# superyuri/FinRL

Hardware: AMD Instinct MI355X
Metric: env-steps/sec at N parallel envs (DOW30, 8 indicators) (higher is better)
Workload: dtype f64

## Files before the change

### finrl_amd/csrc/finenv_stock.hip

```cpp

#include "finenv_stock_common.h"

namespace {

constexpr int kAssetBatch = 16;
template <typename P>
__device__ __forceinline__ double end_total_asset(const P &p, const double *close, int E, int N, int e)
{
    const double *prow = close + (size_t)SI(FINENV_SI_PRICE_DAY) * N;
    double s = 0.0;
    for (int i0 = 0; i0 < N; i0 += kAssetBatch) {
        double pr[kAssetBatch];
        int hd[kAssetBatch];
#pragma unroll
        for (int j = 0; j < kAssetBatch; ++j) {
            const int i = min(i0 + j, N - 1);
            pr[j] = prow[i];
            hd[j] = HOLD(i);
        }
#pragma unroll
        for (int j = 0; j < kAssetBatch; ++j) {
            pin(pr[j]);
            pin(hd[j]);
        }
// ... 93 lines not shown
                    const int el = (N == 1) ? f : (int)__umulhi((unsigned)f, p.magicN);
                    const int kk = ks[el];
                    if (kk >= 1) p.h.actions[((size_t)(kk - 1) * E + e0) * N + f] = v[j];
                }
            }
        }
    }
    if (k >= 1) {
        p.h.asset[(size_t)k * E + e] = end_total_asset(p, p.close, E, N, e);
        p.h.row[(size_t)k * E + e] = SI(FINENV_SI_DAY);
        p.h.len[e] = k + 1;
    }
}

__global__ void stock_history_arm_kernel(const HistoryArgs p)
{
    const int E = p.E, N = p.N;
    const int e = blockIdx.x * blockDim.x + threadIdx.x;
    if (e >= E || (p.mask != nullptr && p.mask[e] == 0)) return;
    p.h.asset[e] = SI(FINENV_SI_DAY) == SI(FINENV_SI_START_DAY) ? SF(FINENV_SF_ASSET0)
                                                                : end_total_asset(p, p.close, E, N, e);
    p.h.row[e] = SI(FINENV_SI_DAY);
    p.h.len[e] = 1;
    p.h.flags[e] = 0;
}

}

struct finenv_stock : finenv_host::Handle {
    finenv_stock_config cfg;
    finenv_stock_panel panel;
    finenv_stock_state st;
    int obs_pitch;
    int desync_hint;
    uint32_t magicN;
    double *last;
    int32_t *win;
    int has_hist;
    finenv_stock_history hist;
    finenv_stock_impl::StepPlan plan;
};

namespace {

Params make_params(const finenv_stock *h)
{
    Params p;
    memset(&p, 0, sizeof(p));
    p.cfg = h->cfg;
    p.panel = h->panel;
    p.st = h->st;
    p.D = h->D;
    p.obs_pitch = h->obs_pitch;
    p.desync_hint = h->desync_hint;
    p.magicN = h->magicN;
    p.last = h->last;
    p.win = h->win;
    return p;
}

int launch_aux(finenv_stock *h, const Params &p, int mode, hipStream_t stream)
{
    if (h->cfg.n_tickers <= 32) finenv_stock_impl::launch_aux_np32(p, mode, stream);
    else if (h->cfg.n_tickers <= 64) finenv_stock_impl::launch_aux_np64(p, mode, stream);
    else finenv_stock_impl::launch_aux_np128(p, mode, stream);
    return 0;
}

void plan_step(finenv_stock *h)
{
    const bool win = h->win != nullptr, desync = h->desync_hint != 0;
    const int N = h->cfg.n_tickers;
    finenv_stock_impl::StepPlan &pl = h->plan;
    pl = N <= 32   ? finenv_stock_impl::choose_step_np32(h->cfg, win, desync)
         : N <= 64 ? finenv_stock_impl::choose_step_np64(h->cfg, win, desync)
                   : finenv_stock_impl::choose_step_np128(h->cfg, win, desync);
    const void *fn = reinterpret_cast<const void *>(pl.kernel);
    const finenv_host::DeviceGuard guard(h->device);
    int dev = h->device, cus = 0, per_cu = 0;
    if (dev < 0) (void)hipGetDevice(&dev);
    pl.lds_refused = pl.lds_bytes > 64 * 1024 &&
                     hipFuncSetAttribute(fn, hipFuncAttributeMaxDynamicSharedMemorySize, (int)pl.lds_bytes) != hipSuccess;
    if (hipDeviceGetAttribute(&cus, hipDeviceAttributeMultiprocessorCount, dev) != hipSuccess || cus < 1) cus = 256;
    if (hipOccupancyMaxActiveBlocksPerMultiprocessor(&per_cu, fn, kStepThreads, pl.lds_bytes) != hipSuccess || per_cu < 1)
        per_cu = 1;
    (void)hipGetLastError();
    pl.round = per_cu * cus;
}

void launch_step_rounds(const finenv_stock_impl::StepPlan &pl, const Params &p, hipStream_t stream)
{
    const int blocks = (p.cfg.n_envs + kWave - 1) / kWave;
    const int k = (blocks + pl.round - 1) / pl.round;
    const int chunk = k > 1 ? (blocks + k - 1) / k : blocks;
    Params q = p;
    int b = 0;
    do {
        q.block_base = b;
        const int nb = blocks - b < chunk ? blocks - b : chunk;
        hipLaunchKernelGGL(pl.kernel, dim3((unsigned)nb), dim3(kStepThreads), pl.lds_bytes, stream, q);
        b += chunk;
    } while (b < blocks);
}

HistoryArgs make_history_args(const finenv_stock *h)
{
    HistoryArgs a;
    memset(&a, 0, sizeof(a));
    a.h = h->hist;
    a.st = h->st;
    a.close = h->panel.close;
    a.E = h->cfg.n_envs;
    a.N = h->cfg.n_tickers;
    a.magicN = h->magicN;
    return a;
}

void launch_history_arm(const finenv_stock *h, const uint8_t *mask, hipStream_t stream)
{
    HistoryArgs a = make_history_args(h);
    a.mask = mask;
    hipLaunchKernelGGL(stock_history_arm_kernel, dim3((a.E + 255) / 256), dim3(256), 0, stream, a);
}

finenv_host::HistorySeries history_series(const finenv_stock *h)
{
    return {h->hist.asset, nullptr, nullptr, h->hist.len, h->hist.flags, 0, h->hist.capacity, h->cfg.n_envs};
}

}

#ifdef FINENV_DIAG
unsigned long long *g_finenv_dbg = nullptr;
#define g_dbg g_finenv_dbg
extern "C" void finenv_diag_set_stamp_buffer(void *ptr) { g_finenv_dbg = (unsigned long long *)ptr; }
#endif

extern "C" {

int finenv_abi_version(void) { return FINENV_ABI_VERSION; }

int finenv_struct_size(int which)
{
    switch (which) {
    case 0: return (int)sizeof(finenv_stock_config);
    case 1: return (int)sizeof(finenv_stock_panel);
    case 2: return (int)sizeof(finenv_stock_state);
    case 3: return (int)sizeof(finenv_portfolio_config);
    case 4: return (int)sizeof(finenv_portfolio_panel);
    case 5: return (int)sizeof(finenv_portfolio_state);
    case 6: return (int)sizeof(finenv_crypto_config);
    case 7: return (int)sizeof(finenv_crypto_panel);
    case 8: return (int)sizeof(finenv_crypto_state);
    case 9: return (int)sizeof(finenv_stocknp_config);
    case 10: return (int)sizeof(finenv_stocknp_panel);
    case 11: return (int)sizeof(finenv_stocknp_state);
    case 12: return (int)sizeof(finenv_cashpenalty_config);
    case 13: return (int)sizeof(finenv_cashpenalty_panel);
    case 14: return (int)sizeof(finenv_cashpenalty_state);
    case 15: return (int)sizeof(finenv_stoploss_config);
    case 16: return (int)sizeof(finenv_stoploss_panel);
    case 17: return (int)sizeof(finenv_stoploss_state);
    case 19: return (int)sizeof(finenv_btc_config);
    case 20: return (int)sizeof(finenv_btc_panel);
    case 21: return (int)sizeof(finenv_btc_state);
    case 23: return (int)sizeof(finenv_replay_view);
    case 24: return (int)sizeof(finenv_replay_batch);
    case 26: return (int)sizeof(finenv_replay_nstep);
    case 28: return (int)sizeof(finenv_replay_per);
    case 30: return (int)sizeof(finenv_rollout_view);
    case 31: return (int)sizeof(finenv_rollout_batch);
    case 33: return (int)sizeof(finenv_vecnorm);
    default: return FINENV_ERR_INVALID;
    }
}

const char *finenv_strerror(int code)
{
    switch (code) {
    case FINENV_OK: return "ok";
    case FINENV_ERR_INVALID: return "invalid argument";
    case FINENV_ERR_UNBOUND: return "panel/state not bound";
    case FINENV_ERR_HIP: return "HIP runtime error";
// ... 229 lines not shown
```

### finrl_amd/csrc/finenv_stock_common.h

```cpp
#pragma once
#include <hip/hip_runtime.h>
#include <stdint.h>
#include <stdio.h>
#include <stdlib.h>
#include <string.h>

#include <cstddef>
#include <new>
#include <type_traits>

#include "finenv.h"
#include "finenv_dev.h"
#include "finenv_host.h"

namespace finenv_stock_impl {
struct Params {
    finenv_stock_config cfg;
    finenv_stock_panel panel;
    finenv_stock_state st;
    const float *actions;
    float *obs;
    float *reward;
    uint8_t *done;
    float *term_obs;
    int32_t *realised;
    const uint8_t *mask;
    double *stats_out;
    int32_t auto_reset;
    int32_t D;
    int32_t obs_pitch;
    int32_t desync_hint;
    int32_t day0;
    uint32_t magicN;
    int32_t block_base;
    int32_t diag;
    unsigned long long *dbg;
    double *last;
    const int32_t *win;
};
}

namespace {

constexpr int kWave = 64;
constexpr int kStepThreads = 2 * kWave;

using finenv_stock_impl::Params;

#ifdef FINENV_DIAG
#define DIAG(bit) (p.diag & (bit))
#define STAMP(k)                                                                          \
    do {                                                                                  \
        if (p.dbg != nullptr && lane == 0) {                                              \
            __builtin_amdgcn_sched_barrier(0);                                            \
            p.dbg[((size_t)(blockIdx.x + p.block_base) * 2 + role) * 16 + (k)] = __builtin_amdgcn_s_memrealtime(); \
            __builtin_amdgcn_sched_barrier(0);                                            \
        }                                                                                 \
    } while (0)
#else
#define DIAG(bit) 0
#define STAMP(k) do { } while (0)
#endif

#define SF(fld) (*at(p.st.f64, (unsigned)(fld) * (unsigned)E + (unsigned)e))
#define SI(fld) (*at(p.st.i32, (unsigned)(fld) * (unsigned)E + (unsigned)e))
#define HOLD(i) SI(FINENV_STOCK_I32_FIELDS + (i))
#define SH0(i) SI(FINENV_STOCK_I32_FIELDS + N + (i))
#define SL(fld) (*at(p.last, (unsigned)(fld) * (unsigned)E + (unsigned)e))

__device__ __forceinline__ void latch_last_episode(const Params &p, double *last, int E, int e,
                                                   double end_asset)
{
#define LB(fld) (*at(last, (unsigned)(fld) * (unsigned)E + (unsigned)e))
    LB(FINENV_SL_COUNT) = LB(FINENV_SL_COUNT) + 1.0;
    LB(FINENV_SL_EPISODE) = (double)SI(FINENV_SI_EPISODE);
    LB(FINENV_SL_BEGIN_ASSET) = SF(FINENV_SF_ASSET0);
    LB(FINENV_SL_END_ASSET) = end_asset;
    LB(FINENV_SL_COST) = SF(FINENV_SF_COST);
    LB(FINENV_SL_TRADES) = (double)SI(FINENV_SI_TRADES);
    LB(FINENV_SL_RET_N) = (double)(SI(FINENV_SI_DAY) - SI(FINENV_SI_START_DAY));
    LB(FINENV_SL_RET_SUM) = SF(FINENV_SF_RET_SUM);
    LB(FINENV_SL_RET_SUMSQ) = SF(FINENV_SF_RET_SUMSQ);
#undef LB
}

__device__ __forceinline__ double *last_block()
{
    const char *ka = (const char *)__builtin_amdgcn_kernarg_segment_ptr();
    asm volatile("" : "+s"(ka));
    return *reinterpret_cast<double *const *>(ka + offsetof(Params, last));
}


__device__ __forceinline__ void ce(int &a, int &b)
{
    const int lo = min(a, b);
    const int hi = max(a, b);
    a = lo;
    b = hi;
}

}

namespace finenv_stock_impl {
struct StepPlan {
    void (*kernel)(Params);
    size_t lds_bytes;
    int round;
    int lds_refused;
};
StepPlan choose_step_np32(const finenv_stock_config &cfg, bool win, bool desync);
StepPlan choose_step_np64(const finenv_stock_config &cfg, bool win, bool desync);
StepPlan choose_step_np128(const finenv_stock_config &cfg, bool win, bool desync);
void launch_aux_np32(const Params &p, int mode, hipStream_t stream);
void launch_aux_np64(const Params &p, int mode, hipStream_t stream);
void launch_aux_np128(const Params &p, int mode, hipStream_t stream);
}
```

### finrl_amd/csrc/finenv_stock_kernels.inc

```

constexpr int kNPad = FINENV_NP;
constexpr int kLog2NPad = FINENV_LOG2NP;
constexpr bool kWide = kNPad > 32;
constexpr int kRow = kNPad + 1;
constexpr int kAuxWaves = kWide ? 1 : 4;
constexpr int kLdsPerWave = kWave * kRow;
constexpr int kAMax = kWide ? 1 << 23 : 1 << 25;
static_assert((long long)kAMax * kNPad + kNPad <= (1ll << 31), "keys must fit int32");
static_assert((1 << kLog2NPad) == kNPad, "NP must be a power of two");

__device__ __forceinline__ void sort_keys(int (&k)[kNPad])
{
#define CE(i, j) ce(k[i], k[j]);
#include FINENV_SORTNET
#undef CE
}


__device__ __forceinline__ double floordiv_exact(double a, double d)
{
    double x = __builtin_amdgcn_rcp(d);
    x = fma(fma(-d, x, 1.0), x, x);
    double q = floor(a * x);
    const double r = fma(-q, d, a);
// ... 148 lines not shown
        }
        for (int k = k_lo; k < nchunk; ++k) {
            const int col = k * kWave + lane;
            const int hidx = col - 1 - N;
            const bool in = col < D;
            const bool patch = in && (col == 0 || (hidx >= 0 && hidx < N));
            const int sel = (col == 0) ? 0 : (patch ? 1 + hidx : 0);
            const bool any_patch = __any(patch);
            for (int g = 0; g < nenv_w; g += kRows) {
                if (((lane_mask >> g) & 0xFFFFFFFFull) == 0ull) continue;
                float t[kRows];
#pragma unroll
                for (int j = 0; j < kRows; ++j) {
                    const int rd = __builtin_amdgcn_readlane(row_day, min(g + j, nenv_w - 1));
                    t[j] = *at(tmpl, (unsigned)(rd * D + (in ? col : 0)));
                }
#pragma unroll
                for (int j = 0; j < kRows; ++j) pin(t[j]);
#pragma unroll
                for (int j = 0; j < kRows; ++j) {
                    const int el = g + j;
                    if (el >= nenv_w || !((lane_mask >> el) & 1ull)) continue;
                    float v = t[j];
                    if (any_patch) {
                        const float pv = pfn(el, sel);
                        v = patch ? pv : v;
                    }
                    if (in) *at(base, (unsigned)(el * P + col)) = v;
                }
            }
        }
        return;
    }
    for (int k = k_lo; k < nchunk; ++k) {
        const int col = k * kWave + lane;
        const bool in = col < D;
        const int hidx = col - 1 - N;
        const bool patch = in && (col == 0 || (hidx >= 0 && hidx < N));
        const int sel = (col == 0) ? 0 : (patch ? 1 + hidx : 0);
        const bool any_patch = __any(patch);
        {
            const float t = in ? *at(tmpl, (unsigned)(rd0 * D + col)) : 0.0f;
            if (all_rows && !any_patch) {
#pragma unroll 8
                for (int el = 0; el < nenv_w; ++el)
                    if (in) *at(base, (unsigned)(el * P + col)) = t;
            } else if (all_rows) {
#pragma unroll 8
                for (int el = 0; el < nenv_w; ++el) {
                    const float pv = pfn(el, sel);
                    if (in) *at(base, (unsigned)(el * P + col)) = patch ? pv : t;
                }
            } else {
                for (int el = 0; el < nenv_w; ++el) {
                    if (!((lane_mask >> el) & 1ull)) continue;
                    const float pv = pfn(el, sel);
                    if (in) *at(base, (unsigned)(el * P + col)) = patch ? pv : t;
                }
            }
        }
    }
}

template <int kDesyncCh = 1>
__device__ __forceinline__ void write_obs_rows(float *__restrict__ dst,
                                               const float *__restrict__ tmpl, int D, int P, int N,
                                               int e0, int nenv_w, int row_day,
                                               unsigned long long lane_mask,
                                               const float *rows, int lane, int k_lo = 0,
                                               int k_hi = 1 << 30, int el_lo = 0,
                                               int el_hi = kWave)
{
    write_obs_rows_fn<kDesyncCh>(dst, tmpl, D, P, N, e0, nenv_w, row_day, lane_mask,
                      [rows](int el, int sel) { return rows[el * kRow + sel]; }, lane, k_lo, k_hi,
                      el_lo, el_hi);
}

constexpr int kR1 = kWave * kRow;
constexpr int kPStride = kWave + 1;
constexpr int kR2 = kWide ? kNPad * 4 : kNPad * kPStride * 2;
constexpr int kR3 = kWave * kRow;
constexpr int kHeadMax = (2 * kNPad) / kWave + 1;
constexpr int kR4 = kHeadMax * kWave;
constexpr int kLdsStep = kR1 + kR2 + kR3 + kR4;

template <bool TURB, bool STATS, bool DES = false, bool WIN = false>
__global__ void __launch_bounds__(kStepThreads, kWide ? 1 : 2)
stock_step_kernel(const Params p)
{
    extern __shared__ __attribute__((aligned(16))) float lds_all[];
    const int lane = threadIdx.x & (kWave - 1);
    const int role = threadIdx.x >> 6;
    float *lds = lds_all;
    int *ldsh = reinterpret_cast<int *>(lds_all);
    double *ldsp = reinterpret_cast<double *>(lds_all + kR1);
    int *ldsk = reinterpret_cast<int *>(lds_all + kR1 + kR2);
    float *rows = lds_all + kR1 + kR2;
    float *ldshead = lds_all + kR1 + kR2 + kR3;
    float *tile = kWide ? rows : lds_all;

    const int E = p.cfg.n_envs, N = p.cfg.n_tickers, D = p.D, T = p.cfg.n_days;
    const int P = p.obs_pitch;
    const int e0 = ((int)blockIdx.x + p.block_base) * kWave;
    if (e0 >= E) return;
    const int nenv_w = min(kWave, E - e0);
    const bool valid = lane < nenv_w;
    const int e = valid ? e0 + lane : e0;

    STAMP(0);
#ifdef FINENV_DIAG
    if (p.dbg != nullptr && lane == 0) p.dbg[((size_t)blockIdx.x * 2 + role) * 16 + 14] = __builtin_amdgcn_s_memtime();
#endif
    const float *__restrict__ act_src = p.actions + (size_t)e0 * N;
    const int act_total = nenv_w * N;
    const int act_n4 = act_total >> 2;
    constexpr int kTileLoads = kWide ? kNPad / 8 : kNPad / 4;
    float4 av[kTileLoads];
    if (kWide || role == 0) {
#pragma unroll
        for (int j = 0; j < kTileLoads; ++j) {
            const int idx4 = (kWide ? 2 * j + role : j) * kWave + lane;
            av[j] = reinterpret_cast<const float4 *>(act_src)[(idx4 < act_n4 && !DIAG(8)) ? idx4 : 0];
        }
    }
    int day = SI(FINENV_SI_DAY);
    int pd = SI(FINENV_SI_PRICE_DAY);
    const int last_day = WIN ? win_last_day(p.win, E, e, T) : T - 1;
    const bool term = day >= last_day;
    const bool do_reset = term && p.auto_reset != 0;
    const int pd_cur = pd;
    const int pd_next = term ? pd : day + 1;
    int reset_row = 0;
    if (WIN && !p.cfg.reset_quirk && __any(do_reset)) reset_row = win_start(p.win, e, T);
    const int row_obs = do_reset ? (p.cfg.reset_quirk ? pd : reset_row) : pd_next;
    const unsigned long long valid_mask = __ballot(valid);
    const unsigned long long term_mask = __ballot(term && valid);
    const int kpatch = (2 * N) / kWave + 1;
    const int ro_first = __builtin_amdgcn_readfirstlane(row_obs);
    auto head_widx = [N](int col) {
        const int hidx = col - 1 - N;
        return col == 0 ? 0 : ((hidx >= 0 && hidx < N) ? 1 + hidx : -1);
    };
    const int pd_first = __builtin_amdgcn_readfirstlane(pd_cur);
    const bool uniform_pd = kWide && __all(pd_cur == pd_first);
    const bool shared_row = !kWide && __all(pd_cur == pd_first);
    const bool desync_days = !__all(pd_cur == pd_first);
    const bool gather_rows = DES && !kWide && desync_days;
    const bool park_heads = gather_rows && kpatch == 1 && D >= kWave;
    typedef float hf4 __attribute__((ext_vector_type(4)));
    typedef hf4 hf4u __attribute__((aligned(4)));
    auto head_rows_parked = [&](const float *park, const float *img, int el_lo, int el_hi) {
        const int w = head_widx(lane);
        float *const hb = p.obs + (size_t)e0 * P;
        for (int g = el_lo; g < el_hi; g += 8) {
            float v[8];
#pragma unroll
            for (int j = 0; j < 8; ++j) {
                const float hv = img[(g + j) * kRow + (w >= 0 ? w : 0)];
                const float pv = park[(g + j) * kWave + lane];
                v[j] = w >= 0 ? hv : pv;
            }
#pragma unroll
            for (int j = 0; j < 8; ++j)
                if (g + j < nenv_w && ((valid_mask >> (g + j)) & 1ull))
                    *at(hb, (unsigned)((g + j) * P + lane)) = v[j];
        }
    };
    const int pmul = shared_row ? 1 : (gather_rows ? kPStride : kWave), padd = shared_row ? 0 : lane;
    const int pn_first = __builtin_amdgcn_readfirstlane(pd_next);
    const bool uniform_next = kWide && __all(pd_next == pn_first);
    STAMP(1);

    double cash = 0.0, cost = 0.0, turb = 0.0, last_reward = 0.0, begin = 0.0;
    double st_mean = 0.0, st_m2 = 0.0;
    int trades = 0;
    bool first_step = false;
    int hreg[kWide ? 1 : kNPad];

    if (role == 0) {
        cash = SF(FINENV_SF_CASH);
        begin = SF(FINENV_SF_BEGIN_ASSET);
        cost = SF(FINENV_SF_COST);
        trades = SI(FINENV_SI_TRADES);
        last_reward = SF(FINENV_SF_LAST_REWARD);
        if (TURB) turb = SF(FINENV_SF_TURBULENCE);
        if (STATS) {
            first_step = day == SI(FINENV_SI_START_DAY);
            st_mean = SF(FINENV_SF_RET_SUM);
            st_m2 = SF(FINENV_SF_RET_SUMSQ);
        }
        if (!kWide) {
#pragma unroll
            for (int i = 0; i < kNPad; ++i) {
                const int hv = HOLD(i < N ? i : 0);
                hreg[i] = (i < N) ? hv : 0;
            }
        }
    }
    if (role == ((kWide || gather_rows) ? 1 : 0)) {
        float head_tt[kHeadMax];
        if (!park_heads) head_fetch(head_tt, p.panel.obs_tmpl, D, ro_first, lane, kpatch);
        if (shared_row) {
            const int i = lane & (kNPad - 1);
            const double pv = *at(p.panel.close, (unsigned)(pd_first * N + (i < N ? i : 0)));
            if (lane < kNPad) ldsp[i] = pv;
        } else if (gather_rows) {
            {
                const int l32 = lane & (kNPad - 1);
                const int li = l32 < N ? l32 : 0;
                double pv[kWave];
#pragma unroll
                for (int j = 0; j < kWave; ++j) {
                    const int de = __builtin_amdgcn_readlane(pd_cur, j);
                    pv[j] = *at(p.panel.close, (unsigned)(de * N + li));
                }
#pragma unroll
                for (int j = 0; j < kWave; ++j)
                    if (lane < kNPad) ldsp[lane * kPStride + j] = pv[j];
            }
        } else if (!kWide) {
            for (int base = 0; base < kNPad; base += 32) {
                double pv[32];
#pragma unroll
                for (int i = 0; i < 32; ++i)
                    pv[i] = *at(p.panel.close,
                                (unsigned)(pd_cur * N + (base + i < N ? base + i : 0)));
#pragma unroll
                for (int i = 0; i < 32; ++i)
                    ldsp[(base + i) * kWave + lane] = pv[i];
            }
        } else {
            int hv[kNPad];
#pragma unroll
            for (int i = 0; i < kNPad; ++i) hv[i] = HOLD(i < N ? i : 0);
            constexpr int kHalves = kNPad / kWave > 0 ? kNPad / kWave : 1;
            double pv[kHalves], pn[kHalves];
#pragma unroll
            for (int half = 0; half < kNPad / kWave; ++half) {
                const int i = half * kWave + lane, ic = i < N ? i : 0;
                pv[half] = *at(p.panel.close, (unsigned)(pd_first * N + ic));
                pn[half] = *at(p.panel.close, (unsigned)(pn_first * N + ic));
            }
#pragma unroll
            for (int half = 0; half < kNPad / kWave; ++half) {
                const int i = half * kWave + lane;
                ldsp[i] = (i < N) ? pv[half] : 0.0;
                ldsp[kNPad + i] = (i < N) ? fabs(pn[half]) : 0.0;
            }
#pragma unroll
            for (int i = 0; i < kNPad; ++i) ldsh[i * kWave + lane] = (i < N) ? hv[i] : 0;
        }
        if (!park_heads) head_park(ldshead, head_tt, lane);
    }
    if (gather_rows && role == 0) {
        asm volatile("s_waitcnt vmcnt(0)" ::: "memory");
        lds_barrier();
    }
    if (kWide || role == 0) {
#pragma unroll
    for (int j = 0; j < kTileLoads; ++j) {
        const int idx4 = (kWide ? 2 * j + role : j) * kWave + lane;
        if (idx4 < act_n4) {
            const float c[4] = {av[j].x, av[j].y, av[j].z, av[j].w};
#pragma unroll
            for (int u = 0; u < 4; ++u) {
                const int f = 4 * idx4 + u;
                const int el = (N == 1) ? f : (int)__umulhi((unsigned)f, p.magicN);
                tile[el * kRow + (f - el * N)] = c[u];
            }
        }
    }
    }
    if (role == (kWide ? 1 : 0))
        for (int f = 4 * act_n4 + lane; f < act_total; f += kWave) {
            const int el = (N == 1) ? f : (int)__umulhi((unsigned)f, p.magicN);
            tile[el * kRow + (f - el * N)] = *at(act_src, (unsigned)f);
        }
    STAMP(2);
    hf4 ht[16];
    if (role == 1 && park_heads) {
        const int q = lane & 15, rs = lane >> 4;
#pragma unroll
        for (int u = 0; u < 16; ++u) {
            const int rd = __shfl(row_obs, min(4 * u + rs, nenv_w - 1));
            ht[u] = *reinterpret_cast<const hf4u *>(reinterpret_cast<const char *>(p.panel.obs_tmpl) +
                                                    (size_t)((unsigned)(rd * D + 4 * q) * 4u));
        }
    }
    if (gather_rows) {
        if (role == 1) lds_barrier(); else wave_sync();
    } else if (!kWide) {
        wave_sync();
    } else {
        lds_barrier();
    }
    STAMP(3);

    if (role == 1) {
        if (!DIAG(1)) {
            if (term_mask != 0ull && p.term_obs != nullptr)
                write_obs_rows(p.term_obs, p.panel.obs_tmpl, D, D, N, e0, nenv_w, pd_cur,
                               term_mask, lds, lane, kpatch);
            constexpr int kDesyncCh = 4;
            write_obs_rows<(DES ? kDesyncCh : 1)>(p.obs, p.panel.obs_tmpl, D, P, N, e0, nenv_w, row_obs, valid_mask, lds,
                              lane, kpatch);
        }
        STAMP(4);
        lds_barrier();
        if (park_heads) {
            float *const park = reinterpret_cast<float *>(ldsp);
            const int q = lane & 15, rs = lane >> 4;
#pragma unroll
            for (int u = 0; u < 16; ++u)
                *reinterpret_cast<hf4 *>(park + (4 * u + rs) * kWave + 4 * q) = ht[u];
            lds_barrier();
            if (!DIAG(1)) head_rows_parked(park, rows, kWave / 2, kWave);
        } else
        if (!DIAG(1) && (term_mask == 0ull || (DES && desync_days))) {
            HeadPlan<kHeadMax> hp;
            head_plan(hp, ldshead, D, row_obs, ro_first, valid_mask, lane, kpatch, head_widx);
            if (hp.uniform)
                head_store(hp, p.obs, D, P, e0, nenv_w, valid_mask, lane, kWave / 2, kWave,
                           [rows](int el, int w) { return rows[el * kRow + w]; });
            else
                write_obs_rows(p.obs, p.panel.obs_tmpl, D, P, N, e0, nenv_w, row_obs, valid_mask,
                               rows, lane, 0, kpatch, kWave / 2, kWave);
        }
        STAMP(5);
        if (valid) {
#pragma unroll 8
            for (int i = 0; i < N; ++i) HOLD(i) = ldsh[i * kWave + lane];
        }
        return;
    }

    if (!kWide) __builtin_amdgcn_s_setprio(3);
    const bool turbulent = TURB && (turb >= p.cfg.turbulence_threshold);
    const int hmax = p.cfg.hmax;
    const float hmaxf = (float)hmax;
    double risk_next = 0.0;
    if (TURB) risk_next = *at(p.panel.risk, (unsigned)pd_next);

    int keys[kNPad];
#pragma unroll
    for (int i = 0; i < kNPad; ++i) {
        const float x = tile[lane * kRow + i] * hmaxf;
        int a = (int)x;
        a = max(-kAMax, min(kAMax, a));
        a = turbulent ? -hmax : a;
        a = (term || i >= N) ? 0 : a;
        keys[i] = a * kNPad + i;
    }
    wave_sync();

    auto price_signed = [&](int idx) -> double {
        if (!kWide) return ldsp[idx * pmul + padd];
        if (uniform_pd) return ldsp[idx];
        return *at(p.panel.close, (unsigned)(pd_cur * N + min(idx, N - 1)));
    };

    double s = 0.0;
    if (!kWide) {
#pragma unroll
        for (int i = 0; i < kNPad; ++i) ldsh[i * kWave + lane] = hreg[i];
    }
    STAMP(4);

    if (!DIAG(4)) sort_keys(keys);
    const double c_s = p.cfg.sell_cost_pct, c_b = p.cfg.buy_cost_pct;
    const double one_m_cs = 1 - c_s, one_p_cb = 1 + c_b;
    const int *kcol = ldsk + lane;
    int *hcol = ldsh + lane;
    double nreg[kWide ? 1 : kNPad];

    if (!kWide) {
        double pS[kNPad];
        int hS[kNPad];
#pragma unroll
        for (int r = 0; r < kNPad; ++r) {
            const int idx = keys[r] & (kNPad - 1);
            pS[r] = ldsp[idx * pmul + padd];
            hS[r] = hcol[idx * kWave];
        }
        STAMP(5);
        if (!DIAG(2)) {
            int n_sold = 0;
#pragma unroll
            for (int g = 0; g < kNPad; g += 4) {
                if (g >= 8 && !__any(keys[g] < 0)) break;
#pragma unroll
                for (int r = g; r < g + 4; ++r) {
                    const int key = keys[r];
                    const int h = hS[r];
                    const int phi = __double2hiint(pS[r]);
                    int m = (key & -h) >> 31;
                    if (TURB) {
                        const int nz = (fabs(pS[r]) > 0.0) ? -1 : 0;
                        m &= turbulent ? nz : ~(phi >> 31);
                    } else {
                        m &= ~(phi >> 31);
                    }
                    int q = min(-(key >> kLog2NPad), h);
                    if (TURB) q = turbulent ? h : q;
                    q &= m;
                    n_sold -= m;
                    const double amt = fabs(pS[r]) * (double)q;
                    cash = cash + amt * one_m_cs;
                    cost = cost + amt * c_s;
                    hcol[(key & (kNPad - 1)) * kWave] = h - q;
                }
            }
            trades += n_sold;
        }
#pragma unroll
        for (int r = 0; r < kNPad; ++r) {
            ldsk[r * kWave + lane] = keys[r];
            ldsp[r * kWave + lane] = pS[r];
        }
        STAMP(6);
        asm volatile("" ::: "memory");
#pragma unroll
        for (int i = 0; i < kNPad; ++i)
            nreg[i] = *at(p.panel.close, (unsigned)(pd_next * N + (i < N ? i : 0)));
        if (!DIAG(2)) {
            auto refined_rcp = [](double u) {
                const double x = __builtin_amdgcn_rcp(u);
                return fma(fma(-u, x, 1.0), x, x);
            };
            const double *pcol = ldsp + lane;
            int key0 = kcol[(kNPad - 1) * kWave], key1 = kcol[(kNPad - 2) * kWave];
            int key2 = kcol[(kNPad - 3) * kWave];
            double p0 = pcol[(kNPad - 1) * kWave], p1 = pcol[(kNPad - 2) * kWave];
            double p2 = pcol[(kNPad - 3) * kWave];
            double u0 = p0 * one_p_cb;
            double x0 = refined_rcp(u0);
#pragma unroll 3
            for (int r = kNPad - 1; r >= 0; --r) {
                if (!__any(key0 >= kNPad)) break;
                const int key3 = kcol[max(r - 3, 0) * kWave];
                const double p3 = pcol[max(r - 3, 0) * kWave];
                const double u1 = p1 * one_p_cb;
                const double x1 = refined_rcp(u1);

                const int idx = key0 & (kNPad - 1);
                const int a0 = key0 >> kLog2NPad;
                const double ad = (double)a0;
                const bool ok = key0 >= kNPad && !turbulent && u0 > 0.0;
                double q0;
                {
                    const double f = floor(cash * x0);
                    asm("v_min_f64 %0, %1, %2" : "=v"(q0) : "v"(f), "v"(ad));
                }
                const double rem = fma(-q0, u0, cash);
                int qi = (int)q0;
                qi += ((rem >= u0) & (qi < a0)) ? 1 : 0;
                qi -= (rem < 0.0) ? 1 : 0;
                qi = ok ? qi : 0;
                const double amt = p0 * (double)qi;
                cash = cash - amt * one_p_cb;
                cost = cost + amt * c_b;
                trades += ok ? 1 : 0;
                __hip_atomic_fetch_add(&hcol[idx * kWave], qi, __ATOMIC_RELAXED,
                                       __HIP_MEMORY_SCOPE_WAVEFRONT);
                key0 = key1; key1 = key2; key2 = key3;
                p0 = p1; p1 = p2; p2 = p3; u0 = u1; x0 = x1;
            }
        }
    } else {
#pragma unroll
    for (int r = 0; r < kNPad; ++r) ldsk[r * kWave + lane] = keys[r];
    STAMP(5);

    if (uniform_pd) {
        if (!DIAG(2)) {
            int n_sold = 0;
            for (int c = 0; c < kNPad; c += 32) {
                if (!__any(kcol[c * kWave] < 0)) break;
                int kk[32], hS[32];
                double pS[32];
#pragma unroll
                for (int r = 0; r < 32; ++r) kk[r] = kcol[(c + r) * kWave];
#pragma unroll
                for (int r = 0; r < 32; ++r) {
                    const int idx = kk[r] & (kNPad - 1);
                    pS[r] = ldsp[idx];
                    hS[r] = hcol[idx * kWave];
                }
#pragma unroll
                for (int r = 0; r < 32; ++r) {
                    const int key = kk[r];
                    const int h = hS[r];
                    const int phi = __double2hiint(pS[r]);
                    int m = (key & -h) >> 31;
                    if (TURB) {
                        const int nz = (fabs(pS[r]) > 0.0) ? -1 : 0;
                        m &= turbulent ? nz : ~(phi >> 31);
                    } else {
                        m &= ~(phi >> 31);
                    }
                    int q = min(-(key >> kLog2NPad), h);
                    if (TURB) q = turbulent ? h : q;
                    q &= m;
                    n_sold -= m;
                    const double amt = fabs(pS[r]) * (double)q;
                    cash = cash + amt * one_m_cs;
                    cost = cost + amt * c_s;
// ... 171 lines not shown
        if (p.term_obs != nullptr)
            write_obs_rows(p.term_obs, p.panel.obs_tmpl, D, D, N, e0, nenv_w, pd_cur, term_mask,
                           rows, lane, 0, kpatch);
        if (p.auto_reset) {
            wave_sync();
            if (term) {
                pd = row_obs;
                cash = SF(FINENV_SF_CASH0);
                for (int i = 0; i < N; ++i) {
                    const int v = SH0(i);
                    hcol[i * kWave] = v;
                    rows[lane * kRow + 1 + i] = (float)v;
                }
                rows[lane * kRow] = (float)cash;
                const double a0 = initial_asset_lds(cash, hcol, p.panel.close, (unsigned)(pd * N),
                                                    N, p.cfg.initial != 0);
                if (p.cfg.single_ticker && p.cfg.initial) {
                    hcol[0] = 0;
                    rows[lane * kRow + 1] = 0.0f;
                }
                end_carry = initial_asset_lds(cash, hcol, p.panel.close, (unsigned)(pd * N), N, false);
                day = WIN ? win_start(p.win, e, T) : 0;
                if (valid) {
                    SF(FINENV_SF_ASSET0) = a0;
                    SF(FINENV_SF_RET_SUM) = 0.0;
                    SF(FINENV_SF_RET_SUMSQ) = 0.0;
                    SI(FINENV_SI_START_DAY) = day;
                }
                turb = 0.0;
                cost = 0.0;
                trades = 0;
                episode_inc = 1;
            }
            wave_sync();
        }
    }

    lds_barrier();
    if (park_heads) lds_barrier();
    HeadPlan<kHeadMax> hpt;
    const bool split_head = term_mask == 0ull || (DES && desync_days);
    if (split_head && !park_heads)
        head_plan(hpt, ldshead, D, row_obs, ro_first, valid_mask, lane, kpatch, head_widx);
    if (!DIAG(1) && !split_head && !park_heads)
        write_obs_rows(p.obs, p.panel.obs_tmpl, D, P, N, e0, nenv_w, row_obs, valid_mask, rows, lane,
                       0, kpatch);
    STAMP(10);

    if (STATS && !term) {
        double st_prev = begin;
        if (__any(first_step)) {
            const double a0 = SF(FINENV_SF_ASSET0);
            st_prev = first_step ? a0 : begin;
        }
        const double ret = end / st_prev - 1.0;
        if (valid) {
            SF(FINENV_SF_RET_SUM) = st_mean + ret;
            SF(FINENV_SF_RET_SUMSQ) = st_m2 + ret * ret;
        }
    }
    if (valid) {
        SF(FINENV_SF_CASH) = cash;
        SF(FINENV_SF_BEGIN_ASSET) = end_carry;
        SF(FINENV_SF_COST) = cost;
        SI(FINENV_SI_TRADES) = trades;
        SI(FINENV_SI_DAY) = day;
        SI(FINENV_SI_PRICE_DAY) = pd;
        SF(FINENV_SF_LAST_REWARD) = last_reward;
        if (TURB) SF(FINENV_SF_TURBULENCE) = turb;
        if (episode_inc) SI(FINENV_SI_EPISODE) += 1;
    }
    if (park_heads) {
        if (!DIAG(1)) head_rows_parked(reinterpret_cast<const float *>(ldsp), rows, 0, kWave / 2);
    } else if (split_head && !DIAG(1)) {
        if (hpt.uniform)
            head_store(hpt, p.obs, D, P, e0, nenv_w, valid_mask, lane, 0, kWave / 2,
                       [rows](int el, int w) { return rows[el * kRow + w]; });
        else
            write_obs_rows(p.obs, p.panel.obs_tmpl, D, P, N, e0, nenv_w, row_obs, valid_mask, rows, lane,
                           0, kpatch, 0, kWave / 2);
    }
    STAMP(11);
#ifdef FINENV_DIAG
    if (p.dbg != nullptr && lane == 0) p.dbg[((size_t)blockIdx.x * 2 + role) * 16 + 15] = __builtin_amdgcn_s_memtime();
#endif
}

__global__ void __launch_bounds__(kWave *kAuxWaves) stock_aux_kernel(const Params p, int mode)
{
    __shared__ float lds_all[kAuxWaves * kLdsPerWave];
    const int lane = threadIdx.x & (kWave - 1);
    const int wib = threadIdx.x >> 6;
    float *lds = lds_all + wib * kLdsPerWave;
    const int E = p.cfg.n_envs, N = p.cfg.n_tickers, D = p.D, P = p.obs_pitch, T = p.cfg.n_days;
    const int e0 = (blockIdx.x * kAuxWaves + wib) * kWave;
    if (e0 >= E) return;
    const int nenv_w = min(kWave, E - e0);
    const bool valid = lane < nenv_w;
    const int e = valid ? e0 + lane : e0;

    int hf[kNPad];
    double cash;
    int pd, start = 0;
    bool sel = valid;
    if (mode >= 2) {
        cash = SF(FINENV_SF_CASH);
        pd = SI(FINENV_SI_PRICE_DAY);
#pragma unroll
        for (int i = 0; i < kNPad; ++i) {
            const int v = HOLD(i < N ? i : 0);
            hf[i] = (i < N) ? v : 0;
        }
        if (mode == 3) {
            const double b0 = initial_asset(cash, hf, p.panel.close + (size_t)pd * N, N, false);
            if (valid) SF(FINENV_SF_BEGIN_ASSET) = b0;
            return;
        }
    } else {
        if (mode == 1 && p.mask != nullptr) sel = valid && p.mask[e] != 0;
        const int w0 = p.win != nullptr ? win_start(p.win, e, T) : 0;
        start = mode == 0 ? min(w0 + p.day0, T - 1) : w0;
        if (mode == 0) pd = start;
        else pd = p.cfg.reset_quirk ? SI(FINENV_SI_PRICE_DAY) : start;
        cash = SF(FINENV_SF_CASH0);
#pragma unroll
        for (int i = 0; i < kNPad; ++i) {
            const int v = SH0(i < N ? i : 0);
            hf[i] = (i < N) ? v : 0;
        }
        const double a0 =
            initial_asset(cash, hf, p.panel.close + (size_t)pd * N, N, p.cfg.initial != 0);
        if (p.cfg.single_ticker && p.cfg.initial) hf[0] = 0;
        const double b0 = initial_asset(cash, hf, p.panel.close + (size_t)pd * N, N, false);
        if (sel) {
            SF(FINENV_SF_CASH) = cash;
            SF(FINENV_SF_BEGIN_ASSET) = b0;
#pragma unroll
            for (int i = 0; i < kNPad; ++i)
                if (i < N) HOLD(i) = hf[i];
            SF(FINENV_SF_ASSET0) = a0;
            SF(FINENV_SF_RET_SUM) = 0.0;
            SF(FINENV_SF_RET_SUMSQ) = 0.0;
            SI(FINENV_SI_START_DAY) = start;
            SI(FINENV_SI_DAY) = start;
            SI(FINENV_SI_PRICE_DAY) = pd;
            SF(FINENV_SF_TURBULENCE) = 0.0;
            SF(FINENV_SF_COST) = 0.0;
            SI(FINENV_SI_TRADES) = 0;
            if (mode == 0) {
                SI(FINENV_SI_EPISODE) = 0;
                SF(FINENV_SF_LAST_REWARD) = 0.0;
            } else {
                SI(FINENV_SI_EPISODE) += 1;
            }
        }
    }
    if (mode == 0 || p.obs == nullptr) return;
    lds[lane * kRow] = (float)cash;
#pragma unroll
    for (int i = 0; i < kNPad; ++i)
        if (i < N) lds[lane * kRow + 1 + i] = (float)hf[i];
    wave_sync();
    write_obs_rows(p.obs, p.panel.obs_tmpl, D, P, N, e0, nenv_w, pd, __ballot(sel), lds, lane);
}
```

### finrl_amd/csrc/finenv_stock_wide.inc

```

typedef float wide_f4 __attribute__((ext_vector_type(4)));

template <int NT>
struct WideGeom {
    static constexpr int kHS = kWave + 1;
    static constexpr int kH = NT * kHS;
    static constexpr int kC = kHS;
    static constexpr int kPOff = (kH + kC + 1) & ~1;
    static constexpr int kP = 4 * NT;
    static constexpr int kKOff = (kPOff + kP + 3) & ~3;
    static constexpr int kK = NT * kWave / 2;
    static constexpr int kDwords = kKOff + kK;
    static constexpr size_t kBytes = sizeof(float) * kDwords;
    static constexpr int kMaxHmax = (32767 - 127) / 128;
};

template <int NT>
__device__ __forceinline__ void sort_keys_pruned(int (&k)[NT])
{
#define CE(i, j) if constexpr ((j) < NT) ce(k[i], k[j]);
#include "sortnet128.inc"
#undef CE
}

template <bool TURB, bool STATS, int NT, bool WIN = false>
__global__ void __launch_bounds__(kStepThreads, 2)
stock_step_wide_kernel(const Params p)
{
    static_assert(NT > 64 && NT <= 128 && NT % 4 == 0, "wide kernel: 64 < NT <= 128, NT % 4 == 0");
    using G = WideGeom<NT>;
    constexpr int kHS = G::kHS;
    extern __shared__ __attribute__((aligned(16))) float lds_all[];
    int *ldsh = reinterpret_cast<int *>(lds_all);
    float *ldsc = lds_all + G::kH;
    double *ldsp = reinterpret_cast<double *>(lds_all + G::kPOff);
    short *ldsk = reinterpret_cast<short *>(lds_all + G::kKOff);
    wide_f4 *ldst = reinterpret_cast<wide_f4 *>(lds_all + G::kKOff);
    const int lane = threadIdx.x & (kWave - 1);
    const int role = __builtin_amdgcn_readfirstlane(threadIdx.x >> 6);

    constexpr int N = NT;
    constexpr int kHoldSplit = NT / 2;
    const int E = p.cfg.n_envs, D = p.D, T = p.cfg.n_days, P = p.obs_pitch;
    const int e0 = ((int)blockIdx.x + p.block_base) * kWave;
    if (e0 >= E) return;
    const int nenv_w = min(kWave, E - e0);
    const bool valid = lane < nenv_w;
    const int e = valid ? e0 + lane : e0;

    STAMP(0);
#ifdef FINENV_DIAG
    if (p.dbg != nullptr && lane == 0) p.dbg[((size_t)blockIdx.x * 2 + role) * 16 + 14] = __builtin_amdgcn_s_memtime();
    if (p.dbg != nullptr && lane == 0)
        p.dbg[((size_t)blockIdx.x * 2 + role) * 16 + 13] =
            (unsigned long long)(__builtin_amdgcn_s_getreg((31 << 11) | 20) & 0xff) |
            ((unsigned long long)__builtin_amdgcn_s_getreg((31 << 11) | 4) << 8);
#endif
    constexpr int kTileLoads = NT / 4;
    constexpr int kHalves = (NT + kWave - 1) / kWave;
    const int act_n4 = nenv_w * (NT / 4);
    wide_f4 av[kTileLoads];
    int hv[NT];
    double pv[kHalves], pn[kHalves];
    if (role == 0) {
#pragma unroll
        for (int i = 0; i < NT; ++i) hv[i] = HOLD(i);
#pragma unroll
        for (int j = 0; j < kTileLoads; ++j) {
            const int idx4 = j * kWave + lane;
            av[j] = *reinterpret_cast<const wide_f4 *>(
                at(p.actions, (unsigned)(e0 * NT + 4 * (idx4 < act_n4 ? idx4 : 0))));
        }
    }
    int day = SI(FINENV_SI_DAY);
    int pd = SI(FINENV_SI_PRICE_DAY);
    const int last_day = WIN ? win_last_day(p.win, E, e, T) : T - 1;
    const bool term = day >= last_day;
    const bool do_reset = term && p.auto_reset != 0;
    const int pd_cur = pd;
    const int pd_next = term ? pd : day + 1;
    int reset_row = 0;
    if (WIN && !p.cfg.reset_quirk && __any(do_reset)) reset_row = win_start(p.win, e, T);
    const int row_obs = do_reset ? (p.cfg.reset_quirk ? pd : reset_row) : pd_next;
    const unsigned long long valid_mask = __ballot(valid);
    const unsigned long long term_mask = __ballot(term && valid);
    constexpr int kpatch = (2 * N) / kWave + 1;
    const int pd_first = __builtin_amdgcn_readfirstlane(pd_cur);
    const bool uniform_pd = __all(pd_cur == pd_first);
    const int pn_first = __builtin_amdgcn_readfirstlane(pd_next);
    const bool uniform_next = __all(pd_next == pn_first);
    if (role == 0) {
#pragma unroll
        for (int half = 0; half < kHalves; ++half) {
            const int i = half * kWave + lane, ic = i < N ? i : 0;
            pv[half] = *at(p.panel.close, (unsigned)(pd_first * N + ic));
            pn[half] = *at(p.panel.close, (unsigned)(pn_first * N + ic));
        }
    }
    STAMP(1);

    auto patch = [ldsh](int el, int sel) -> float {
        const int bits = ldsh[(sel == 0 ? NT : sel - 1) * kHS + el];
        return sel == 0 ? __int_as_float(bits) : (float)bits;
    };
    auto head_widx = [](int col) {
        const int hidx = col - 1 - NT;
        return col == 0 ? NT * kHS : ((hidx >= 0 && hidx < NT) ? hidx * kHS : -1);
    };
    auto head_val = [ldsh](int el, int w) -> float {
        const int bits = ldsh[w + el];
        return w == NT * kHS ? __int_as_float(bits) : (float)bits;
    };
    HeadPlan<kpatch> hp;
    const int ro_first = __builtin_amdgcn_readfirstlane(row_obs);
    float *ldshead = lds_all + G::kKOff;

    if (role == 1) {
        STAMP(2);
        STAMP(3);
        if (!DIAG(1)) {
#pragma nounroll
            for (int pass = (term_mask != 0ull && p.term_obs != nullptr) ? 0 : 1; pass < 2; ++pass)
                write_obs_rows(pass == 0 ? p.term_obs : p.obs, p.panel.obs_tmpl, D, pass == 0 ? D : P, N, e0, nenv_w,
                               pass == 0 ? pd_cur : row_obs, pass == 0 ? term_mask : valid_mask,
                               lds_all, lane, kpatch);
        }
        STAMP(4);
        lds_barrier();
        if (valid) {
#pragma unroll 10
            for (int i = kHoldSplit; i < N; ++i) HOLD(i) = ldsh[i * kHS + lane];
        }
        return;
    }

    double cash = SF(FINENV_SF_CASH);
    const double begin = SF(FINENV_SF_BEGIN_ASSET);
// ... 305 lines not shown
                    SF(FINENV_SF_RET_SUM) = 0.0;
                    SF(FINENV_SF_RET_SUMSQ) = 0.0;
                    SI(FINENV_SI_START_DAY) = day;
                }
                turb = 0.0;
                cost = 0.0;
                trades = 0;
                episode_inc = 1;
            }
            wave_sync();
        }
    }

    const bool quad_rows = kQuadHead && D >= kpatch * kWave &&
                           __all(!valid || row_obs == ro_first);
    wave_sync();
    if (!quad_rows) {
        head_park(ldshead, head_tt, lane);
        wave_sync();
        head_plan(hp, ldshead, D, row_obs, ro_first, valid_mask, lane, kpatch, head_widx);
    }
    if (quad_rows && !DIAG(1)) {
        int w[4];
#pragma unroll
        for (int u = 0; u < 4; ++u) w[u] = head_widx(4 * lane + u);
        char *const hb = reinterpret_cast<char *>(p.obs + (size_t)e0 * P);
        constexpr int kB = 8;
        for (int g = 0; g < nenv_w; g += kB) {
            float pv4[kB][4];
#pragma unroll
            for (int j = 0; j < kB; ++j)
#pragma unroll
                for (int u = 0; u < 4; ++u)
                    pv4[j][u] = head_val(min(g + j, kWave - 1), w[u] >= 0 ? w[u] : 0);
#pragma unroll
            for (int j = 0; j < kB; ++j) {
                const int el = g + j;
                if (el >= nenv_w) continue;
                wide_f4 v;
#pragma unroll
                for (int u = 0; u < 4; ++u) v[u] = w[u] >= 0 ? pv4[j][u] : head_q[u];
                *reinterpret_cast<wide_f4u *>(hb + (size_t)((unsigned)(el * P + 4 * lane) * 4u)) = v;
            }
        }
    }
    if (!DIAG(1) && !quad_rows) {
        if (hp.uniform)
            head_store(hp, p.obs, D, P, e0, nenv_w, valid_mask, lane, 0, kWave, head_val);
        else
            write_obs_rows_fn(p.obs, p.panel.obs_tmpl, D, P, N, e0, nenv_w, row_obs, valid_mask, patch,
                              lane, 0, kpatch, 0, kWave);
    }
    lds_barrier();
    if (valid) {
        SF(FINENV_SF_CASH) = cash;
        SF(FINENV_SF_BEGIN_ASSET) = end_carry;
        SF(FINENV_SF_COST) = cost;
        SI(FINENV_SI_TRADES) = trades;
        SI(FINENV_SI_DAY) = day;
        SI(FINENV_SI_PRICE_DAY) = pd;
        SF(FINENV_SF_LAST_REWARD) = last_reward;
        if (TURB) SF(FINENV_SF_TURBULENCE) = turb;
        if (episode_inc) SI(FINENV_SI_EPISODE) += 1;
    }
    if (STATS && !term) {
        double st_prev = begin;
        if (__any(first_step)) {
            const double a0 = SF(FINENV_SF_ASSET0);
            st_prev = first_step ? a0 : begin;
        }
        const double ret = end / st_prev - 1.0;
        if (valid) {
            SF(FINENV_SF_RET_SUM) = st_mean + ret;
            SF(FINENV_SF_RET_SUMSQ) = st_m2 + ret * ret;
        }
    }
    if (valid) {
#pragma unroll 10
        for (int i = 0; i < kHoldSplit; ++i) HOLD(i) = hcol[i * kHS];
    }
    STAMP(10);
    STAMP(11);
#ifdef FINENV_DIAG
    if (p.dbg != nullptr && lane == 0) p.dbg[((size_t)blockIdx.x * 2 + role) * 16 + 15] = __builtin_amdgcn_s_memtime();
#endif
}
```

### finrl_amd/csrc/finenv_stock_width.inc

```
#include "finenv_stock_common.h"

#define FINENV_CAT_(a, b) a##b
#define FINENV_CAT(a, b) FINENV_CAT_(a, b)
#define FINENV_WIDTH_NS FINENV_CAT(np, FINENV_NP)

namespace {
namespace FINENV_WIDTH_NS {
#include "finenv_stock_kernels.inc"
#include "finenv_stock_wide.inc"

template <bool TURB, bool STATS>
finenv_stock_impl::StepPlan choose_step(const finenv_stock_config &cfg, bool win, bool desync)
{
    constexpr size_t lds = sizeof(float) * kLdsStep;
    if constexpr (!kWide) {
        if (win) return {stock_step_kernel<TURB, STATS, true, true>, lds};
        if (desync) return {stock_step_kernel<TURB, STATS, true, false>, lds};
    } else {
        if constexpr (kNPad == 128) {
            using G = WideGeom<100>;
            if (cfg.n_tickers == 100 && cfg.hmax <= G::kMaxHmax)
                return win ? finenv_stock_impl::StepPlan{stock_step_wide_kernel<TURB, STATS, 100, true>, G::kBytes}
                           : finenv_stock_impl::StepPlan{stock_step_wide_kernel<TURB, STATS, 100, false>, G::kBytes};
        }
        if (win) return {stock_step_kernel<TURB, STATS, false, true>, lds};
    }
    return {stock_step_kernel<TURB, STATS, false, false>, lds};
}
}
}

namespace finenv_stock_impl {

StepPlan FINENV_CAT(choose_step_np, FINENV_NP)(const finenv_stock_config &cfg, bool win, bool desync)
{
    using namespace FINENV_WIDTH_NS;
    const bool turb = cfg.use_turbulence != 0, stats = cfg.track_stats != 0;
    if (turb && stats) return choose_step<true, true>(cfg, win, desync);
    if (turb) return choose_step<true, false>(cfg, win, desync);
    if (stats) return choose_step<false, true>(cfg, win, desync);
    return choose_step<false, false>(cfg, win, desync);
}

void FINENV_CAT(launch_aux_np, FINENV_NP)(const Params &p, int mode, hipStream_t stream)
{
    using namespace FINENV_WIDTH_NS;
    const int waves = (p.cfg.n_envs + kWave - 1) / kWave;
    const dim3 grid((unsigned)((waves + kAuxWaves - 1) / kAuxWaves));
    hipLaunchKernelGGL(stock_aux_kernel, grid, dim3(kWave * kAuxWaves), 0, stream, p, mode);
}

}
```

Measured before the change: 3.338 billion.

## Add a dedicated sorter wave to overlap action sorting with step work

Result: faster. 3.563 billion (median of 6 runs) (+6.7%).

```diff
diff --git a/finrl_amd/csrc/finenv_stock.hip b/finrl_amd/csrc/finenv_stock.hip
--- a/finrl_amd/csrc/finenv_stock.hip
+++ b/finrl_amd/csrc/finenv_stock.hip
@@ -199,7 +199,7 @@
     pl.lds_refused = pl.lds_bytes > 64 * 1024 &&
                      hipFuncSetAttribute(fn, hipFuncAttributeMaxDynamicSharedMemorySize, (int)pl.lds_bytes) != hipSuccess;
     if (hipDeviceGetAttribute(&cus, hipDeviceAttributeMultiprocessorCount, dev) != hipSuccess || cus < 1) cus = 256;
-    if (hipOccupancyMaxActiveBlocksPerMultiprocessor(&per_cu, fn, kStepThreads, pl.lds_bytes) != hipSuccess || per_cu < 1)
+    if (hipOccupancyMaxActiveBlocksPerMultiprocessor(&per_cu, fn, pl.threads, pl.lds_bytes) != hipSuccess || per_cu < 1)
         per_cu = 1;
     (void)hipGetLastError();
     pl.round = per_cu * cus;
@@ -215,7 +215,7 @@
     do {
         q.block_base = b;
         const int nb = blocks - b < chunk ? blocks - b : chunk;
-        hipLaunchKernelGGL(pl.kernel, dim3((unsigned)nb), dim3(kStepThreads), pl.lds_bytes, stream, q);
+        hipLaunchKernelGGL(pl.kernel, dim3((unsigned)nb), dim3((unsigned)pl.threads), pl.lds_bytes, stream, q);
         b += chunk;
     } while (b < blocks);
 }
diff --git a/finrl_amd/csrc/finenv_stock_common.h b/finrl_amd/csrc/finenv_stock_common.h
--- a/finrl_amd/csrc/finenv_stock_common.h
+++ b/finrl_amd/csrc/finenv_stock_common.h
@@ -44,6 +44,7 @@
 
 constexpr int kWave = 64;
 constexpr int kStepThreads = 2 * kWave;
+constexpr int kStampRoles = 3;
 
 using finenv_stock_impl::Params;
 
@@ -53,7 +54,7 @@
     do {                                                                                  \
         if (p.dbg != nullptr && lane == 0) {                                              \
             __builtin_amdgcn_sched_barrier(0);                                            \
-            p.dbg[((size_t)(blockIdx.x + p.block_base) * 2 + role) * 16 + (k)] = __builtin_amdgcn_s_memrealtime(); \
+            p.dbg[((size_t)(blockIdx.x + p.block_base) * kStampRoles + role) * 16 + (k)] = __builtin_amdgcn_s_memrealtime(); \
             __builtin_amdgcn_sched_barrier(0);                                            \
         }                                                                                 \
     } while (0)
@@ -106,6 +107,7 @@
 struct StepPlan {
     void (*kernel)(Params);
     size_t lds_bytes;
+    int threads = kStepThreads;
     int round;
     int lds_refused;
 };
diff --git a/finrl_amd/csrc/finenv_stock_kernels.inc b/finrl_amd/csrc/finenv_stock_kernels.inc
--- a/finrl_amd/csrc/finenv_stock_kernels.inc
+++ b/finrl_amd/csrc/finenv_stock_kernels.inc
@@ -254,21 +254,132 @@
 constexpr int kR3 = kWave * kRow;
 constexpr int kHeadMax = (2 * kNPad) / kWave + 1;
 constexpr int kR4 = kHeadMax * kWave;
-constexpr int kLdsStep = kR1 + kR2 + kR3 + kR4;
+constexpr int kR5 = kWide ? 0 : 4;
+constexpr int kLdsStep = kR1 + kR2 + kR3 + kR4 + kR5;
+
+__device__ __forceinline__ void scatter_quad(float *tile, const float4 &v, int idx4, int N, unsigned magicN)
+{
+    const float c[4] = {v.x, v.y, v.z, v.w};
+#pragma unroll
+    for (int u = 0; u < 4; ++u) {
+        const int f = 4 * idx4 + u;
+        const int el = (N == 1) ? f : (int)__umulhi((unsigned)f, magicN);
+        tile[el * kRow + (f - el * N)] = c[u];
+    }
+}
+__device__ __forceinline__ void scatter_leftover(float *tile, const float *__restrict__ act_src, int act_n4,
+                                                 int act_total, int N, unsigned magicN, int lane)
+{
+    for (int f = 4 * act_n4 + lane; f < act_total; f += kWave) {
+        const int el = (N == 1) ? f : (int)__umulhi((unsigned)f, magicN);
+        tile[el * kRow + (f - el * N)] = *at(act_src, (unsigned)f);
+    }
+}
+
+__device__ __forceinline__ void build_keys(int (&keys)[kNPad], const float *tile, int lane, int N, int hmax,
+                                           bool turbulent, bool term)
+{
+    const float hmaxf = (float)hmax;
+#pragma unroll
+    for (int i = 0; i < kNPad; ++i) {
+        const float x = tile[lane * kRow + i] * hmaxf;
+        int a = (int)x;
+        a = max(-kAMax, min(kAMax, a));
+        a = turbulent ? -hmax : a;
+        a = (term || i >= N) ? 0 : a;
+        keys[i] = a * kNPad + i;
+    }
+}
+
+template <bool DES>
+constexpr bool kThreeWave = !kWide && !DES;
+#ifndef FINENV_SORTER_PRIO
+#define FINENV_SORTER_PRIO 3
+#endif
+#ifndef FINENV_SORTER_ROWS
+#define FINENV_SORTER_ROWS 16
+#endif
+constexpr int kSorterRow0 = kWave - FINENV_SORTER_ROWS;
+template <bool DES>
+constexpr int kBlockThreads = kThreeWave<DES> ? 3 * kWave : kStepThreads;
+
+__device__ __forceinline__ void flag_barrier()
+{
+    __builtin_amdgcn_sched_barrier(0);
+    lds_barrier();
+    __builtin_amdgcn_sched_barrier(0);
+}
+
+template <bool TURB, bool WIN>
+__device__ __forceinline__ void sorter_wave(const Params &p, float *tile, int *ldsk, int *sort_flag,
+                                            const float *act_src, int e0, int nenv_w, int e, int lane)
+{
+    constexpr int role = 2;
+    constexpr int kTileLoads = kNPad / 4;
+    const int E = p.cfg.n_envs, N = p.cfg.n_tickers, T = p.cfg.n_days, D = p.D;
+    const int act_total = nenv_w * N;
+    const int act_n4 = act_total >> 2;
+    float4 av[kTileLoads];
+#pragma unroll
+    for (int j = 0; j < kTileLoads; ++j) {
+        const int idx4 = j * kWave + lane;
+        av[j] = reinterpret_cast<const float4 *>(act_src)[(idx4 < act_n4 && !DIAG(8)) ? idx4 : 0];
+    }
+    const int day = SI(FINENV_SI_DAY);
+    const int pd = SI(FINENV_SI_PRICE_DAY);
+    int wend = T;
+    if (WIN) wend = *at(p.win, (unsigned)E + (unsigned)e);
+    double turb = 0.0;
+    if (TURB) turb = SF(FINENV_SF_TURBULENCE);
+    flag_barrier();
+    __builtin_amdgcn_s_setprio(FINENV_SORTER_PRIO);
+    const int last_day = WIN ? min(max(wend, 1), T) - 1 : T - 1;
+    STAMP(1);
+#pragma unroll
+    for (int j = 0; j < kTileLoads; ++j) {
+        const int idx4 = j * kWave + lane;
+        if (idx4 < act_n4) scatter_quad(tile, av[j], idx4, N, p.magicN);
+    }
+    scatter_leftover(tile, act_src, act_n4, act_total, N, p.magicN, lane);
+    wave_sync();
+    STAMP(2);
+    int keys[kNPad];
+    build_keys(keys, tile, lane, N, p.cfg.hmax, TURB && (turb >= p.cfg.turbulence_threshold), day >= last_day);
+    STAMP(3);
+    if (!DIAG(4)) sort_keys(keys);
+    STAMP(4);
+#pragma unroll
+    for (int r = 0; r < kNPad; ++r) ldsk[r * kWave + lane] = keys[r];
+    __builtin_amdgcn_fence(__ATOMIC_RELEASE, "workgroup");
+    __hip_atomic_store(sort_flag, 1, __ATOMIC_RELAXED, __HIP_MEMORY_SCOPE_WORKGROUP);
+    STAMP(5);
+    __builtin_amdgcn_s_setprio(0);
+    const bool term = day >= last_day;
+    const bool do_reset = term && p.auto_reset != 0;
+    int reset_row = 0;
+    if (WIN && !p.cfg.reset_quirk && __any(do_reset)) reset_row = win_start(p.win, e, T);
+    const int row_obs = do_reset ? (p.cfg.reset_quirk ? pd : reset_row) : (term ? pd : day + 1);
+    if (!DIAG(1))
+        write_obs_rows(p.obs, p.panel.obs_tmpl, D, p.obs_pitch, N, e0, nenv_w, row_obs, __ballot(lane < nenv_w), tile,
+                       lane, (2 * N) / kWave + 1, 1 << 30, kSorterRow0, kWave);
+    STAMP(6);
+}
 
 template <bool TURB, bool STATS, bool DES = false, bool WIN = false>
-__global__ void __launch_bounds__(kStepThreads, kWide ? 1 : 2)
+__global__ void __launch_bounds__(kBlockThreads<DES>, kWide ? 1 : (kThreeWave<DES> ? 3 : 2))
 stock_step_kernel(const Params p)
 {
     extern __shared__ __attribute__((aligned(16))) float lds_all[];
+    constexpr bool kThree = kThreeWave<DES>;
     const int lane = threadIdx.x & (kWave - 1);
-    const int role = threadIdx.x >> 6;
+    const int role = kThree ? __builtin_amdgcn_readfirstlane(threadIdx.x >> 6) : threadIdx.x >> 6;
     float *lds = lds_all;
     int *ldsh = reinterpret_cast<int *>(lds_all);
     double *ldsp = reinterpret_cast<double *>(lds_all + kR1);
     int *ldsk = reinterpret_cast<int *>(lds_all + kR1 + kR2);
     float *rows = lds_all + kR1 + kR2;
     float *ldshead = lds_all + kR1 + kR2 + kR3;
+    int *sort_flag = reinterpret_cast<int *>(lds_all + kR1 + kR2 + kR3 + kR4);
     float *tile = kWide ? rows : lds_all;
 
     const int E = p.cfg.n_envs, N = p.cfg.n_tickers, D = p.D, T = p.cfg.n_days;
@@ -281,14 +392,24 @@
 
     STAMP(0);
 #ifdef FINENV_DIAG
-    if (p.dbg != nullptr && lane == 0) p.dbg[((size_t)blockIdx.x * 2 + role) * 16 + 14] = __builtin_amdgcn_s_memtime();
+    if (p.dbg != nullptr && lane == 0) p.dbg[((size_t)blockIdx.x * kStampRoles + role) * 16 + 14] = __builtin_amdgcn_s_memtime();
+    if (p.dbg != nullptr && lane == 0)
+        p.dbg[((size_t)blockIdx.x * kStampRoles + role) * 16 + 13] =
+            (unsigned long long)(__builtin_amdgcn_s_getreg((31 << 11) | 20) & 0xff) |
+            ((unsigned long long)__builtin_amdgcn_s_getreg((31 << 11) | 4) << 8);
 #endif
     const float *__restrict__ act_src = p.actions + (size_t)e0 * N;
     const int act_total = nenv_w * N;
     const int act_n4 = act_total >> 2;
     constexpr int kTileLoads = kWide ? kNPad / 8 : kNPad / 4;
+    if constexpr (kThree) {
+        if (role == 2) {
+            sorter_wave<TURB, WIN>(p, lds_all, ldsk, sort_flag, act_src, e0, nenv_w, e, lane);
+            return;
+        }
+    }
     float4 av[kTileLoads];
-    if (kWide || role == 0) {
+    if (kWide || (!kThree && role == 0)) {
 #pragma unroll
         for (int j = 0; j < kTileLoads; ++j) {
             const int idx4 = (kWide ? 2 * j + role : j) * kWave + lane;
@@ -298,6 +419,10 @@
     int day = SI(FINENV_SI_DAY);
     int pd = SI(FINENV_SI_PRICE_DAY);
     const int last_day = WIN ? win_last_day(p.win, E, e, T) : T - 1;
+    if constexpr (kThree) {
+        if (role == 0) *sort_flag = 0;
+        flag_barrier();
+    }
     const bool term = day >= last_day;
     const bool do_reset = term && p.auto_reset != 0;
     const int pd_cur = pd;
@@ -428,7 +553,7 @@
         asm volatile("s_waitcnt vmcnt(0)" ::: "memory");
         lds_barrier();
     }
-    if (kWide || role == 0) {
+    if (kWide || (!kThree && role == 0)) {
 #pragma unroll
     for (int j = 0; j < kTileLoads; ++j) {
         const int idx4 = (kWide ? 2 * j + role : j) * kWave + lane;
@@ -443,7 +568,7 @@
         }
     }
     }
-    if (role == (kWide ? 1 : 0))
+    if (!kThree && role == (kWide ? 1 : 0))
         for (int f = 4 * act_n4 + lane; f < act_total; f += kWave) {
             const int el = (N == 1) ? f : (int)__umulhi((unsigned)f, p.magicN);
             tile[el * kRow + (f - el * N)] = *at(act_src, (unsigned)f);
@@ -475,7 +600,7 @@
                                term_mask, lds, lane, kpatch);
             constexpr int kDesyncCh = 4;
             write_obs_rows<(DES ? kDesyncCh : 1)>(p.obs, p.panel.obs_tmpl, D, P, N, e0, nenv_w, row_obs, valid_mask, lds,
-                              lane, kpatch);
+                              lane, kpatch, 1 << 30, 0, kThree ? kSorterRow0 : kWave);
         }
         STAMP(4);
         lds_barrier();
@@ -511,9 +636,10 @@
     const int hmax = p.cfg.hmax;
     const float hmaxf = (float)hmax;
     double risk_next = 0.0;
-    if (TURB) risk_next = *at(p.panel.risk, (unsigned)pd_next);
+    if (TURB && !kThree) risk_next = *at(p.panel.risk, (unsigned)pd_next);
 
     int keys[kNPad];
+    if constexpr (!kThree) {
 #pragma unroll
     for (int i = 0; i < kNPad; ++i) {
         const float x = tile[lane * kRow + i] * hmaxf;
@@ -523,6 +649,7 @@
         a = (term || i >= N) ? 0 : a;
         keys[i] = a * kNPad + i;
     }
+    }
     wave_sync();
 
     auto price_signed = [&](int idx) -> double {
@@ -532,13 +659,24 @@
     };
 
     double s = 0.0;
+    if constexpr (kThree) {
+        STAMP(12);
+        while (__hip_atomic_load(sort_flag, __ATOMIC_RELAXED, __HIP_MEMORY_SCOPE_WORKGROUP) == 0)
+            __builtin_amdgcn_s_sleep(1);
+        __builtin_amdgcn_fence(__ATOMIC_ACQUIRE, "workgroup");
+    }
     if (!kWide) {
 #pragma unroll
         for (int i = 0; i < kNPad; ++i) ldsh[i * kWave + lane] = hreg[i];
     }
     STAMP(4);
 
-    if (!DIAG(4)) sort_keys(keys);
+    if constexpr (kThree) {
+#pragma unroll
+        for (int r = 0; r < kNPad; ++r) keys[r] = ldsk[r * kWave + lane];
+    } else {
+        if (!DIAG(4)) sort_keys(keys);
+    }
     const double c_s = p.cfg.sell_cost_pct, c_b = p.cfg.buy_cost_pct;
     const double one_m_cs = 1 - c_s, one_p_cb = 1 + c_b;
     const int *kcol = ldsk + lane;
@@ -586,7 +724,7 @@
         }
 #pragma unroll
         for (int r = 0; r < kNPad; ++r) {
-            ldsk[r * kWave + lane] = keys[r];
+            if (!kThree) ldsk[r * kWave + lane] = keys[r];
             ldsp[r * kWave + lane] = pS[r];
         }
         STAMP(6);
@@ -594,6 +732,7 @@
 #pragma unroll
         for (int i = 0; i < kNPad; ++i)
             nreg[i] = *at(p.panel.close, (unsigned)(pd_next * N + (i < N ? i : 0)));
+        if (TURB && kThree) risk_next = *at(p.panel.risk, (unsigned)pd_next);
         if (!DIAG(2)) {
             auto refined_rcp = [](double u) {
                 const double x = __builtin_amdgcn_rcp(u);
@@ -931,7 +1070,7 @@
     }
     STAMP(11);
 #ifdef FINENV_DIAG
-    if (p.dbg != nullptr && lane == 0) p.dbg[((size_t)blockIdx.x * 2 + role) * 16 + 15] = __builtin_amdgcn_s_memtime();
+    if (p.dbg != nullptr && lane == 0) p.dbg[((size_t)blockIdx.x * kStampRoles + role) * 16 + 15] = __builtin_amdgcn_s_memtime();
 #endif
 }
 
diff --git a/finrl_amd/csrc/finenv_stock_wide.inc b/finrl_amd/csrc/finenv_stock_wide.inc
--- a/finrl_amd/csrc/finenv_stock_wide.inc
+++ b/finrl_amd/csrc/finenv_stock_wide.inc
@@ -50,9 +50,9 @@
 
     STAMP(0);
 #ifdef FINENV_DIAG
-    if (p.dbg != nullptr && lane == 0) p.dbg[((size_t)blockIdx.x * 2 + role) * 16 + 14] = __builtin_amdgcn_s_memtime();
+    if (p.dbg != nullptr && lane == 0) p.dbg[((size_t)blockIdx.x * kStampRoles + role) * 16 + 14] = __builtin_amdgcn_s_memtime();
     if (p.dbg != nullptr && lane == 0)
-        p.dbg[((size_t)blockIdx.x * 2 + role) * 16 + 13] =
+        p.dbg[((size_t)blockIdx.x * kStampRoles + role) * 16 + 13] =
             (unsigned long long)(__builtin_amdgcn_s_getreg((31 << 11) | 20) & 0xff) |
             ((unsigned long long)__builtin_amdgcn_s_getreg((31 << 11) | 4) << 8);
 #endif
@@ -524,6 +524,6 @@
     STAMP(10);
     STAMP(11);
 #ifdef FINENV_DIAG
-    if (p.dbg != nullptr && lane == 0) p.dbg[((size_t)blockIdx.x * 2 + role) * 16 + 15] = __builtin_amdgcn_s_memtime();
+    if (p.dbg != nullptr && lane == 0) p.dbg[((size_t)blockIdx.x * kStampRoles + role) * 16 + 15] = __builtin_amdgcn_s_memtime();
 #endif
 }
diff --git a/finrl_amd/csrc/finenv_stock_width.inc b/finrl_amd/csrc/finenv_stock_width.inc
--- a/finrl_amd/csrc/finenv_stock_width.inc
+++ b/finrl_amd/csrc/finenv_stock_width.inc
@@ -25,7 +25,7 @@
         }
         if (win) return {stock_step_kernel<TURB, STATS, false, true>, lds};
     }
-    return {stock_step_kernel<TURB, STATS, false, false>, lds};
+    return {stock_step_kernel<TURB, STATS, false, false>, lds, kBlockThreads<false>};
 }
 }
 }
```
